# 66RING/tiny-flash-attention

Hardware: AMD Instinct MI355X
Metric: fwd TFLOPS + achieved %MFMA-roofline, (B=4,H=32,N=4096,D=128) bf16 (higher is better)
Workload: dtype bf16

## Files before the change

tiny-flash-attention_amd/csrc/tfa_fwd_il_epilogue.inc:

```
    if (PREF && !PREF2 && more_passes) issue_prologue(next_mb, true);
    if (SEAM) { seam_in = seam; if (seam) issue_prologue(next_mb, false); }
    typedef __attribute__((address_space(4))) const KArgs kargs_c;
    kargs_c* pe_ = (kargs_c*)__builtin_amdgcn_kernarg_segment_ptr();
    asm volatile("" : "+s"(pe_));
    kargs_c& pe = *pe_;
    VarSeq vse{};
    if constexpr (VARLEN) vse = varlen_seq(pe, b);
    const int lane_e = (int)__builtin_amdgcn_mbcnt_hi(~0u, __builtin_amdgcn_mbcnt_lo(~0u, 0u));
    const int qi_e = lane_e & 31, hi_e = lane_e >> 5, my_row_e = wave_row0 + qi_e;
    float l_tot = pair_sum((l4[0] + l4[1]) + (l4[2] + l4[3]));
    float w0 = 1.f, w1 = 0.f;
    const char* const dump = smem + 4 * TILE_BYTES;
    if constexpr (KSPLIT) {
      float* const ml = reinterpret_cast<float*>(smem + wave * (32 * D * 2)) + lane_e * 2;
      if (grp == 1) {
        ml[0] = mref; ml[1] = l_tot;
#pragma unroll
        for (int d = 0; d < DT; ++d) {
          float o[16];
          if (d == 0) o_read<0>(o, 1.f); else if (d == 1) o_read<1>(o, 1.f); else if (d == 2) o_read<2>(o, 1.f); else o_read<3>(o, 1.f);
#pragma unroll
          for (int g = 0; g < 4; ++g) {
            const f32x4 v4 = {o[4 * g + 0], o[4 * g + 1], o[4 * g + 2], o[4 * g + 3]};
            *reinterpret_cast<f32x4*>(const_cast<char*>(dump) + ((((wave * DT + d) << 2) + g) << 10) + lane_e * 16) = v4;
          }
        }
      }
      asm volatile("s_waitcnt lgkmcnt(0)\n\ts_barrier" ::: "memory");
      if (grp == 1) {
        if (!more_passes) return;
        asm volatile("s_barrier" ::: "memory");
        continue;
      }
      const float m1 = ml[0], l1 = ml[1];
      const float m = fmaxf(mref, m1);
      w0 = (mref == -INFINITY) ? 0.f : fast_exp2(mref - m);
      w1 = (m1 == -INFINITY) ? 0.f : fast_exp2(m1 - m);
      l_tot = w0 * l_tot + w1 * l1;
      mref = m;
    }
    const bool empty = !(l_tot > 0.f);
    const float inv = empty ? 1.f : 1.f / l_tot;
    auto o_get = [&](int d, float (&o)[16]) {
      const float f0 = inv * w0;
      if (d == 0) o_read<0>(o, f0); else if (d == 1) o_read<1>(o, f0); else if (d == 2) o_read<2>(o, f0); else o_read<3>(o, f0);
      if constexpr (KSPLIT) {
        const float f1 = inv * w1;
#pragma unroll
        for (int g = 0; g < 4; ++g) {
          const f32x4 x = *reinterpret_cast<const f32x4*>(dump + ((((wave * DT + d) << 2) + g) << 10) + lane_e * 16);
#pragma unroll
          for (int e = 0; e < 4; ++e) o[4 * g + e] = fmaf(f1, x[e], o[4 * g + e]);
        }
      }
    };
    if (PREF2) {
      const float lse = empty ? INFINITY : (mref + __builtin_amdgcn_logf(l_tot)) * 0.6931471805599453f;
      auto lse_rs = __builtin_amdgcn_make_buffer_rsrc((void*)(VARLEN ? pe.lse + ((long long)h * pe.total_q + vse.q0) : pe.lse + (long long)bh * pe.Nq), 0,
                                                      pe.lse != nullptr ? (unsigned)(VARLEN ? vse.nq : pe.Nq) * 4u : 0u, 0x00020000);
      __builtin_amdgcn_raw_buffer_store_b32(__builtin_bit_cast(unsigned, lse), lse_rs, hi_e == 0 ? my_row_e * 4 : (int)TFA_OOB, 0, 0);
    } else
    if (pe.lse != nullptr && hi_e == 0 && my_row_e < (VARLEN ? vse.nq : pe.Nq)) {
      const float lse = empty ? INFINITY : (mref + __builtin_amdgcn_logf(l_tot)) * 0.6931471805599453f;
      if constexpr (VARLEN) pe.lse[(long long)h * pe.total_q + vse.q0 + my_row_e] = lse;
      else pe.lse[(long long)bh * pe.Nq + my_row_e] = lse;
    }
    if (PREF2 && more_passes && !early_done) {
      asm volatile("" ::: "memory");
      issue_prologue(next_mb, true);
      asm volatile("" ::: "memory");
    }
    if (F32OUT) {
      float* obase = reinterpret_cast<float*>(pe.o) + (VARLEN ? (long long)vse.q0 * pe.os_n : b * pe.os_b) + h * pe.os_h;
      auto o_rs = slice_rsrc(obase, VARLEN ? varlen_bytes(vse.nq, pe.os_n, pe.dv, 4) : pe.o_bytes, (unsigned long long)q0 * (unsigned long long)pe.os_n * 4ull);
      const int ooff = (my_row_e - (WIN ? q0 : 0)) * (int)pe.os_n * 4 + hi_e * 16;
      static_assert(!F32OUT || NST_EPI == DT * 4, "NST_EPI must equal the fp32 epilogue's store count");
#pragma unroll
      for (int d = 0; d < DT; ++d) {
        float o[16];
        o_get(d, o);
#pragma unroll
        for (int g = 0; g < 4; ++g) {
// ... 67 lines not shown
```

tiny-flash-attention_amd/csrc/tfa_fwd_il_pass_prologue.inc:

```
    if (SEAM && seam_in) {  }
    else if (PREF2) {  }
    else if (QLDS && pass == 0) { issue_first(mb); asm volatile("s_setprio 0" ::: "memory"); }
    else if (!PREF || pass == 0) { issue_prologue(mb, true); asm volatile("s_setprio 0" ::: "memory"); }
    const bool seam = SEAM && (pass + 1 < npass) && ((nt & 1) == 0) && nt >= 2;
    if (!PREF2) o_zero<DT>();

    if (PREF2) {
    } else {
#if defined(TFA_IL_TRACEPRO)
      if (P_TRACE && pass == 0) {
        tp_issue = __builtin_amdgcn_s_memtime();
        asm volatile("s_waitcnt vmcnt(%0)" ::"n"(DS) : "memory");
        tp_kv = __builtin_amdgcn_s_memtime();
        asm volatile("s_waitcnt vmcnt(0)" ::: "memory");
        tp_q = __builtin_amdgcn_s_memtime();
      }
#endif
      if (QLDS && pass == 0) { wait_first(); read_q_lds(); }
      else asm volatile("s_waitcnt vmcnt(0)" ::: "memory");
#pragma unroll
      for (int s = 0; s < DS; ++s) asm volatile("" : "+v"(qf[s]));
    }
#if defined(TFA_IL_TRACEPRO)
    if (P_TRACE && pass == 0) tp_bar = __builtin_amdgcn_s_memtime();
#endif
    asm volatile("s_barrier" ::: "memory");
    if (P_TRACE && pass == tr_pass) t_pro = __builtin_amdgcn_s_memtime();

    const int nact = (wave_last_tile + 1 < nt_own) ? (wave_last_tile + 1) : nt_own;
    const bool idle_wave = (VF & VF_IL_IDLE) != 0 && wave_row0 >= p.Nq;
    int fm = nact;
    {
      int first_g = 0x3fffffff;
      if (IL_NK % BN) first_g = IL_NK / BN;
      if (CAUSAL) {
        const int c = pos_lo + shift + 1;
        const int full = c > 0 ? c / BN : 0;
        first_g = full < first_g ? full : first_g;
      }
      const int first = KSPLIT ? (first_g <= grp ? 0 : (first_g - grp + 1) >> 1) : first_g;
      fm = first < fm ? first : fm;
    }

    f32x16 sA[2], sB[2];
    asm volatile("" : "=v"(sA[0]), "=v"(sA[1]), "=v"(sB[0]), "=v"(sB[1]));
    float mA = -INFINITY, mB = -INFINITY;
    auto qk_burst = [&](int kbuf, int t, f32x16 (&s)[2], float& mout) {
#pragma unroll
      for (int tt = 0; tt < 2; ++tt)
#pragma unroll
        for (int r = 0; r < 16; ++r) s[tt][r] = 0.f;
      const unsigned kb = kbuf * TILE_BYTES;
#pragma unroll
      for (int i = 0; i < N1; ++i) s[KT(i)] = E::mfma(k_frag_rt(kb, i), qf[KS(i)], s[KT(i)]);
      if constexpr (SMOD) apply_bias(t, s);
      if (needs_mask(t)) apply_mask(t, s);
      float mx = s[0][0];
#pragma unroll
      for (int tt = 0; tt < 2; ++tt)
#pragma unroll
        for (int r = 0; r < 16; ++r) mx = fmaxf(mx, s[tt][r]);
      mout = pair_max(mx);
    };
    if (nact > 0 && !idle_wave) {
      qk_burst(0, 0, sA, mA);
      mref = fmaxf(mref, mA * sc);
    }
    if constexpr (MAXFREE) {
      if (seeded) {
        const int l_ = (int)__builtin_amdgcn_mbcnt_hi(~0u, __builtin_amdgcn_mbcnt_lo(~0u, 0u));
        mref = fmaxf(mref, reinterpret_cast<volatile float*>(smem + SEED_OFF)[wave_id * 32 + (l_ & 31)]);
      }
    }
    if (QLDS && pass == 0) asm volatile("s_waitcnt vmcnt(0)" ::: "memory");
    asm volatile("s_waitcnt lgkmcnt(0)\n\ts_barrier" ::: "memory");

#if defined(TFA_IL_TRACEWAIT)
    auto iter_end = [&]() {
      const unsigned long long a0 = __builtin_amdgcn_s_memtime();
      asm volatile("s_waitcnt vmcnt(0) lgkmcnt(0)" ::: "memory");
      const unsigned long long a1 = __builtin_amdgcn_s_memtime();
      asm volatile("s_barrier" ::: "memory");
      const unsigned long long a2 = __builtin_amdgcn_s_memtime();
      tw_wait += a1 - a0;
      tw_bar += a2 - a1;
    };
#elif defined(TFA_IL_TRACEITER)
    int it_n = 0;
    auto it_stamp = [&](int tag) {
      if (P_TRACE && pass == tr_pass && it_n < 16) {
        typedef __attribute__((address_space(3))) u32x2 lds_u32x2;
        const u32x2 rec = {(unsigned)__builtin_amdgcn_s_memtime(), (unsigned)tag};
        *reinterpret_cast<lds_u32x2*>(q_slice + it_n * 8) = rec;
        ++it_n;
      }
    };
    it_stamp(0);
    auto iter_end = [&]() { asm volatile("s_waitcnt vmcnt(0) lgkmcnt(0)\n\ts_barrier" ::: "memory"); it_stamp(2); };
#else
    auto iter_end = [&]() { asm volatile("s_waitcnt vmcnt(0) lgkmcnt(0)\n\ts_barrier" ::: "memory"); };
#endif
```

tiny-flash-attention_amd/csrc/tfa_fwd_il_tile_loop.inc:

```
    auto fused = [&](auto par_c, auto mask_c, auto resc_c, float alpha, int j, f32x16 (&scur)[2], f32x16 (&snext)[2], float& mnext) {
      constexpr int PAR = decltype(par_c)::value;
      constexpr bool MASK = decltype(mask_c)::value;
      constexpr bool RESC = decltype(resc_c)::value;
      static_assert(!RESC || N1 * 4 == 16 * DT, "one O register quad per QK^T MFMA");
      constexpr bool SPREAD = (VF & VF_IL_DMASPREAD) != 0;
      constexpr bool STAGGER = SPREAD && (VF & VF_IL_DMASTAGGER) != 0;
      const bool late = STAGGER && wave >= NW / 2;
      const bool issue_k = (j + 2 < nt) || seam;
      const int tk = (j + 2 < nt) ? j + 2 : j + 2 - nt;
      if (!SPREAD && !(AB & ILAB_NODMA)) {
        if (issue_k) dma_k(tk, PAR);
        dma_v(j + 1, PAR ^ 1);
      }
      const float msc = mref;
      constexpr int KB = PAR ^ 1;
      const char* vbp = vl + PAR * TILE_BYTES;
      unsigned pw[16];
      float xs[32];
      X8 kf[N1], vf[N2];
#pragma unroll
      for (int i = 0; i < PFK; ++i) kf[i] = k_frag(KB, i);
      auto soft_slot = [&](int g) {
#pragma unroll
        for (int e = 0; e < 32; ++e) {
// ... 132 lines not shown
        const int nact_s = __builtin_amdgcn_readfirstlane(nact), nt_s = __builtin_amdgcn_readfirstlane(nt);
        const int fmx = __builtin_amdgcn_readfirstlane(tail_on ? fm : -1);
        int ts;
        const int slim = __builtin_amdgcn_readfirstlane(wave_row0 + shift - key0_of(fm));
        constexpr bool BF = std::is_same<T, __bf16>::value;
        if constexpr (MAXFREE) {
          if constexpr (D == 128 && PPW == 2) { TFA_IL_ASM_LAZY_STMT(TFA_IL_ASM_LOOP_MF); }
          else if constexpr (D == 128) { TFA_IL_ASM_LAZY_STMT_G(TFA_IL_ASM_LOOP_D128_P4_MF, TFA_IL_ASM_Q8, TFA_IL_ASM_SRC4); }
          else if constexpr (PPW == 1) { TFA_IL_ASM_LAZY_STMT_G(TFA_IL_ASM_LOOP_D64_P1_MF, TFA_IL_ASM_Q4, TFA_IL_ASM_SRC1); }
          else { TFA_IL_ASM_LAZY_STMT_G(TFA_IL_ASM_LOOP_D64_P2_MF, TFA_IL_ASM_Q4, TFA_IL_ASM_SRC2); }
        }
        else if constexpr (D == 128 && PPW == 2 && BF) { TFA_IL_ASM_LAZY_STMT(TFA_IL_ASM_LOOP); }
        else if constexpr (D == 128 && PPW == 2) { TFA_IL_ASM_LAZY_STMT(TFA_IL_ASM_LOOP_F16); }
        else if constexpr (D == 128 && BF) { TFA_IL_ASM_LAZY_STMT_G(TFA_IL_ASM_LOOP_D128_P4, TFA_IL_ASM_Q8, TFA_IL_ASM_SRC4); }
        else if constexpr (D == 128) { TFA_IL_ASM_LAZY_STMT_G(TFA_IL_ASM_LOOP_D128_P4_F16, TFA_IL_ASM_Q8, TFA_IL_ASM_SRC4); }
        else if constexpr (PPW == 1 && BF) { TFA_IL_ASM_LAZY_STMT_G(TFA_IL_ASM_LOOP_D64_P1, TFA_IL_ASM_Q4, TFA_IL_ASM_SRC1); }
        else if constexpr (PPW == 1) { TFA_IL_ASM_LAZY_STMT_G(TFA_IL_ASM_LOOP_D64_P1_F16, TFA_IL_ASM_Q4, TFA_IL_ASM_SRC1); }
        else if constexpr (BF) { TFA_IL_ASM_LAZY_STMT_G(TFA_IL_ASM_LOOP_D64_P2, TFA_IL_ASM_Q4, TFA_IL_ASM_SRC2); }
        else { TFA_IL_ASM_LAZY_STMT_G(TFA_IL_ASM_LOOP_D64_P2_F16, TFA_IL_ASM_Q4, TFA_IL_ASM_SRC2); }
      }
    };
    auto asm_loop_exact = [&](int& j) {
      if constexpr (ASMLOOPX) {
        const int lim = fm < nact ? fm : nact;
        const int jend = (lim - 1 < nt_full - 2) ? lim - 1 : nt_full - 2;
        int koff = (j + 2) * k_tile_stride, voff = (j + 1) * v_tile_stride;
        const unsigned vaddr = lds_base + (unsigned)v_rd_base;
        const unsigned ldsw = __builtin_amdgcn_readfirstlane(lds_base + wave * (PPW * 1024));
        float alpha;
        u32x4 f0, f1, f2, f3, ka;
        unsigned ka5, ka6, ka7;
        const int nact_s = __builtin_amdgcn_readfirstlane(nact), nt_s = __builtin_amdgcn_readfirstlane(nt);
        const int fmx = __builtin_amdgcn_readfirstlane(tail_on ? fm : -1);
        int ts;
        const int slim = __builtin_amdgcn_readfirstlane(wave_row0 + shift - key0_of(fm));
        if constexpr (std::is_same<T, __bf16>::value) { TFA_IL_ASM_EXACT_STMT(TFA_IL_ASM_LOOP_EXACT); }
        else { TFA_IL_ASM_EXACT_STMT(TFA_IL_ASM_LOOP_EXACT_F16); }
      }
    };
    if (!idle_wave)
#pragma nounroll
    for (int j = 0; j < nact; j += 2) {
      if constexpr (EXACT) {
        if (ASMLOOPX && (loop_ok(j) || tail_on)) {
          int jj = j;
          asm_loop_exact(jj);
          if (jj & 1) j = jj - 1;
          else { j = jj - 2; continue; }
        } else
        if (j + 1 < nact) fast_exact(C0{}, j + 1 >= fm, j, sA, mA, sB, mB);
        else slow(j, sA, mA, sB, mB);
        if (j + 1 >= nact) break;
        if (j + 2 < nact) fast_exact(C1{}, j + 2 >= fm, j + 1, sB, mB, sA, mA);
        else slow(j + 1, sB, mB, sA, mA);
      } else {
      if (ASMLOOP && !trigger(mA) && (loop_ok(j) || tail_on) && (!LOCAL || j + 1 >= nlm)) {
        int jj = j;
        asm_loop(jj, (early_ok && nact == nt) ? 1 : 0);
#if defined(TFA_IL_TRACEITER)
        it_stamp(1 | (jj << 8));
#endif
        if (jj & 1) j = jj - 1;
        else { j = jj - 2; continue; }
      } else
      if (!ASMLOOP && j + 1 < nact && !trigger(mA)) {
        if (SMOD ? !needs_mask(j + 1) : j + 1 < fm) fused(C0{}, MN{}, MN{}, 1.f, j, sA, sB, mB);
        else fused(C0{}, MY{}, MN{}, 1.f, j, sA, sB, mB);
      } else {
        slow(j, sA, mA, sB, mB);
      }
      if (j + 1 >= nact) break;
      if (ASMLOOP && early_ok && nact == nt && j + 1 == nt - 1 && !trigger(mB)) {
        last_pending = true;
        break;
      }
      if (!ASMLOOP && j + 2 < nact && !trigger(mB)) {
        if (SMOD ? !needs_mask(j + 2) : j + 2 < fm) fused(C1{}, MN{}, MN{}, 1.f, j + 1, sB, sA, mA);
        else fused(C1{}, MY{}, MN{}, 1.f, j + 1, sB, sA, mA);
      } else {
        slow(j + 1, sB, mB, sA, mA);
      }
      }
    }
#pragma nounroll
    for (int j = idle_wave ? 0 : (last_pending ? nt - 1 : nact); j < nt; ++j) {
      if (early_ok && j == nt - 1) {
        issue_early(block_of(pass + 1));
        early_done = true;
        if (last_pending) {
          int jj = j;
          asm_loop(jj, 2);
        } else asm volatile("s_waitcnt lgkmcnt(0)\n\ts_barrier" ::: "memory");
#if defined(TFA_IL_TRACEITER)
        it_stamp(2);
#endif
        break;
      }
      if (j + 2 < nt) dma_k(j + 2, j & 1);
      else if (seam) dma_k(j + 2 - nt, j & 1);
      if (j + 1 < nt) dma_v(j + 1, (j & 1) ^ 1);
      else if (seam) dma_v(0, (j & 1) ^ 1);
      iter_end();
    }
    bool redo_pass = false;
    if constexpr (MAXFREE) {
      volatile int* const redo_w = reinterpret_cast<volatile int*>(smem + REDO_OFF);
      const float lt_ = (l4[0] + l4[1]) + (l4[2] + l4[3]);
      if (__any(!(lt_ <= 0x1p64f))) *redo_w = 1;
      asm volatile("s_waitcnt lgkmcnt(0)\n\ts_barrier" ::: "memory");
      redo_pass = __builtin_amdgcn_readfirstlane(*redo_w) != 0 && !seeded;
      seeded = false;
    }
    if (P_TRACE && pass == tr_pass) t_loop = __builtin_amdgcn_s_memtime();
#if defined(TFA_IL_TRACEITER)
    if (P_TRACE && pass == tr_pass && blockIdx.x < 64) {
      typedef __attribute__((address_space(3))) const u32x2 lds_u32x2c;
      it_stamp(3 | (nt << 8) | (nact << 16));
      const int l_ = (int)__builtin_amdgcn_mbcnt_hi(~0u, __builtin_amdgcn_mbcnt_lo(~0u, 0u));
      if (l_ < 16) {
        const u32x2 r_ = *reinterpret_cast<lds_u32x2c*>(q_slice + l_ * 8);
        P_TRACE[(size_t)gridDim.x * 8 + ((size_t)blockIdx.x * 8 + wave_id) * 16 + l_] = l_ < it_n ? (((unsigned long long)r_[1] << 32) | r_[0]) : 0ull;
      }
      asm volatile("s_waitcnt vmcnt(0) lgkmcnt(0)" ::: "memory");
    }
#endif
```

tiny-flash-attention_amd/csrc/tfa_fwd_kernel_il.h:

```cpp
#pragma once
#include <type_traits>
#include "tfa_fwd_kernel_dma.h"

namespace tfa {


constexpr int VF_IL = 32768;
constexpr int VF_IL_DMASPREAD = 65536;
constexpr int VF_IL_EPI = 262144;
constexpr int VF_IL_EPI_INPLACE = 1048576;
constexpr int VF_IL_PREF = 524288;
constexpr int VF_IL_SEAM = 2097152;
constexpr int VF_IL_KSPLIT = 1 << 25;
constexpr int VF_IL_IDLE = 1 << 26;
constexpr bool IL_DECODE_NT = true;
constexpr int IL_OSTORE_AUX = 2;
constexpr int VF_IL_WINDOWED = 1 << 24;
constexpr int VF_IL_PREF2 = 1 << 29;
constexpr int VF_IL_QLDS = 1 << 28;
constexpr int VF_IL_EXACT = 1 << 30;
constexpr int VF_IL_DMASTAGGER = 131072;
constexpr int VF_IL_VARLEN = 1 << 23;
constexpr int VF_IL_LOCAL = 1 << 22;
constexpr int VF_IL_ALIBI = 256;
constexpr int VF_IL_SOFTCAP = 512;

}
#include "tfa_fwd_il_regs.h"
#if defined(TFA_IL_ASM_INC)
#include TFA_IL_ASM_INC
#else
#include "tfa_fwd_il_asm_loop.inc"
#endif
#define TFA_IL_ASM_Q8 [q0] "v"(qf[0]), [q1] "v"(qf[1]), [q2] "v"(qf[2]), [q3] "v"(qf[3]), [q4] "v"(qf[4]), [q5] "v"(qf[5]), [q6] "v"(qf[6]), [q7] "v"(qf[7])
#define TFA_IL_ASM_Q4 [q0] "v"(qf[0]), [q1] "v"(qf[1]), [q2] "v"(qf[2]), [q3] "v"(qf[3])
#define TFA_IL_ASM_SRC1 [ks0] "v"(k_src[0]), [vs0] "v"(v_src[0])
#define TFA_IL_ASM_SRC2 [ks0] "v"(k_src[0]), [ks1] "v"(k_src[1]), [vs0] "v"(v_src[0]), [vs1] "v"(v_src[1])
#define TFA_IL_ASM_SRC4 [ks0] "v"(k_src[0]), [ks1] "v"(k_src[1]), [ks2] "v"(k_src[2]), [ks3] "v"(k_src[3]), [vs0] "v"(v_src[0]), [vs1] "v"(v_src[1]), [vs2] "v"(v_src[2]), [vs3] "v"(v_src[3])
#define TFA_IL_ASM_LAZY_STMT_G(TEXT, QOPS, SRCOPS) \
  asm volatile(TEXT \
  : [sa0] "+v"(sA[0]), [sa1] "+v"(sA[1]), [sb0] "+v"(sB[0]), [sb1] "+v"(sB[1]), \
  [l0] "+v"(l4[0]), [l1] "+v"(l4[1]), [l2] "+v"(l4[2]), [l3] "+v"(l4[3]), [ma] "+v"(mA), [mb] "+v"(mB), [j] "+s"(j), \
  [koff] "+s"(koff), [voff] "+s"(voff), [ts] "=&s"(ts), \
  [f0] "=&v"(f0), [f1] "=&v"(f1), [f2] "=&v"(f2), [f3] "=&v"(f3), [ka] "=&v"(ka), [ka5] "=&v"(ka5), [ka6] "=&v"(ka6), [ka7] "=&v"(ka7), [thr] "=&v"(thr) \
  : QOPS, [mref] "v"(mref), [kaddr] "v"(k_rd_addr), [va] "v"(vaddr), SRCOPS, \
  [sc] "s"(sc), [krs] "s"(k_rs), [vrs] "s"(v_rs), [ldsw] "s"(ldsw), [kstr] "s"(k_tile_stride), [vstr] "s"(v_tile_stride), [jend] "s"(jend), \
  [nact] "s"(nact_s), [fmx] "s"(fmx), [nt] "s"(nt_s), [slim] "s"(slim), [xl] "s"(xl) \
  : TFA_O_CLOB0, TFA_O_CLOB1, TFA_O_CLOB2, TFA_O_CLOB3, "m0", "vcc", "scc", "memory")
#define TFA_IL_ASM_LAZY_STMT(TEXT) TFA_IL_ASM_LAZY_STMT_G(TEXT, TFA_IL_ASM_Q8, TFA_IL_ASM_SRC2)
#define TFA_IL_ASM_EXACT_STMT(TEXT) \
  asm volatile(TEXT \
  : [sa0] "+v"(sA[0]), [sa1] "+v"(sA[1]), [sb0] "+v"(sB[0]), [sb1] "+v"(sB[1]), \
  [l0] "+v"(l4[0]), [l1] "+v"(l4[1]), [l2] "+v"(l4[2]), [l3] "+v"(l4[3]), [ma] "+v"(mA), [mb] "+v"(mB), [mref] "+v"(mref), [j] "+s"(j), \
  [koff] "+s"(koff), [voff] "+s"(voff), [ts] "=&s"(ts), \
  [f0] "=&v"(f0), [f1] "=&v"(f1), [f2] "=&v"(f2), [f3] "=&v"(f3), [ka] "=&v"(ka), [ka5] "=&v"(ka5), [ka6] "=&v"(ka6), [ka7] "=&v"(ka7), [alpha] "=&v"(alpha) \
  : [q0] "v"(qf[0]), [q1] "v"(qf[1]), [q2] "v"(qf[2]), [q3] "v"(qf[3]), [q4] "v"(qf[4]), [q5] "v"(qf[5]), [q6] "v"(qf[6]), [q7] "v"(qf[7]), \
  [kaddr] "v"(k_rd_addr), [va] "v"(vaddr), [ks0] "v"(k_src[0]), [ks1] "v"(k_src[1]), [vs0] "v"(v_src[0]), [vs1] "v"(v_src[1]), \
  [sc] "s"(sc), [krs] "s"(k_rs), [vrs] "s"(v_rs), [ldsw] "s"(ldsw), [kstr] "s"(k_tile_stride), [vstr] "s"(v_tile_stride), [jend] "s"(jend), \
  [nact] "s"(nact_s), [fmx] "s"(fmx), [nt] "s"(nt_s), [slim] "s"(slim) \
  : TFA_O_CLOB0, TFA_O_CLOB1, TFA_O_CLOB2, TFA_O_CLOB3, "m0", "vcc", "scc", "memory")
#if !defined(TFA_IL_USE_ASMTAIL)
#define TFA_IL_USE_ASMTAIL 1
#endif
#if !defined(TFA_IL_USE_EARLY)
#define TFA_IL_USE_EARLY 0
#endif
#if !defined(TFA_IL_USE_MAXFREE)
#define TFA_IL_USE_MAXFREE 1
#endif
#if !defined(TFA_IL_USE_ASMLOOP)
#define TFA_IL_USE_ASMLOOP 1
#endif

#if defined(TFA_IL_PAD)
#define TFA_IL_PAD1_0 asm volatile("s_nop 0");
#define TFA_IL_PAD1_1 { int pad_s_; asm volatile("s_mov_b32 %0, 0" : "=s"(pad_s_)); }
#define TFA_IL_PAD1_2 { int pad_v_; asm volatile("v_mov_b32 %0, 0" : "=v"(pad_v_)); }
#define TFA_IL_PAD1_3 asm volatile("s_waitcnt vmcnt(63) lgkmcnt(15)");
#define TFA_IL_PADCAT_(k) TFA_IL_PAD1_##k
#define TFA_IL_PADCAT(k) TFA_IL_PADCAT_(k)
#define TFA_IL_PAD_HERE { _Pragma("unroll") for (int pad_i_ = 0; pad_i_ < TFA_IL_PAD; ++pad_i_) TFA_IL_PADCAT(TFA_IL_PADKIND) }
#else
#define TFA_IL_PAD_HERE
#endif

namespace tfa {

constexpr int ILAB_TRACE = 256;
#define P_TRACE ((AB & ILAB_TRACE) ? p.trace : (unsigned long long*)nullptr)
constexpr int ILAB_NOEXP = 1, ILAB_NODMA = 2, ILAB_NOBARRIER = 4, ILAB_NOMAX = 8, ILAB_NOQK = 16, ILAB_NOPV = 32, ILAB_NOKREAD = 64, ILAB_NOVREAD = 128;

template <typename T, int D, int NW, bool CAUSAL, bool F32OUT, int VF, int AB = 0, int DVB = D / 32>
__global__ __launch_bounds__(NW * 64, 2) __attribute__((amdgpu_num_vgpr(96))) void fwd_kernel_il(const KArgs p) {
  using E = Elem<T>;
  using X8 = typename E::x8;
  constexpr bool KSPLIT = (VF & VF_IL_KSPLIT) != 0;
  constexpr int NWG = KSPLIT ? NW / 2 : NW;
  constexpr int BM = NWG * 32;
  static_assert(!KSPLIT || ((VF & VF_IL_EPI_INPLACE) && !(VF & (VF_IL_SEAM | VF_IL_PREF | VF_IL_WINDOWED))), "KSPLIT: in-place epilogue");
  constexpr int KSTEP = KSPLIT ? 2 : 1;
  constexpr int BN = 64;
  constexpr int CPR = D / 8;
  constexpr int TILE_BYTES = BN * D * 2;
  constexpr int PIECES = TILE_BYTES / 1024;
  constexpr int PPW = PIECES / NWG;
  static_assert(DVB >= 1 && DVB <= D / 32, "valid 32-column blocks of a D-wide kernel");
  constexpr int DS = 2 * DVB;
  constexpr int DT = DVB;
  constexpr int DT_L = D / 32;
  constexpr int N1 = 2 * DS;
  constexpr int N2 = 4 * DT;
  constexpr int NE1 = 21;
  constexpr int PFK = 2, PFV = 2;
  auto slot_of_elem = [](int e) constexpr -> int {
    return 1 + (e < NE1 ? e * N1 / NE1 : N1 + (e - NE1) * (3 * DT - 1) / (32 - NE1));
  };
  static_assert(slot_of_elem(7) < N1 && slot_of_elem(15) < N1 + DT && slot_of_elem(23) < N1 + 2 * DT && slot_of_elem(31) < N1 + 3 * DT,
                "a P slot is packed too late for the PV MFMA that reads it");
#define KT(i) ((i) & 1)
#define KS(i) ((i) >> 1)
  constexpr bool PAIR = CAUSAL && (VF & VF_PAIR);
  static_assert(PPW >= 1 && PPW * NWG == PIECES, "tile does not split into whole DMA pieces per wave");

  extern __shared__ __attribute__((aligned(1024))) char smem[];
  asm volatile("s_setprio 1" ::: "memory");
  const int wave_id = __builtin_amdgcn_readfirstlane(threadIdx.x >> 6);
  const int grp = KSPLIT ? wave_id / NWG : 0;
  char* const gsm = smem + grp * 4 * TILE_BYTES;
  char* const kl = gsm;
  char* const vl = gsm + 2 * TILE_BYTES;
  const unsigned lds_base = (unsigned)(size_t)(__attribute__((address_space(3))) char*)gsm;

  unsigned long long t_start = 0, t_pro = 0, t_loop = 0, rt_start = 0;
#if defined(TFA_IL_TRACEPRO)
  const unsigned long long tp_entry = __builtin_amdgcn_s_memtime();
#endif
  if (P_TRACE) { rt_start = __builtin_amdgcn_s_memrealtime(); t_start = __builtin_amdgcn_s_memtime(); }
  const int tid = threadIdx.x;
  const int lane = tid & 63;
#if defined(TFA_IL_TRACEPRO)
#define TP_STAMP(k, dep)                                                                                                         \
  do {                                                                                                                             \
    asm volatile("" ::"s"(dep));                                                                                                   \
    if (P_TRACE) {                                                                                                                 \
      const unsigned long long t_ = __builtin_amdgcn_s_memtime();                                                                  \
      P_TRACE[(size_t)gridDim.x * 8 + (size_t)gridDim.x * 32 + ((size_t)blockIdx.x * 8 + wave_id) * 8 + (k)] = t_;  \
    }                                                                                                                              \
  } while (0)
  if (P_TRACE) P_TRACE[(size_t)gridDim.x * 8 + (size_t)gridDim.x * 32 + ((size_t)blockIdx.x * 8 + wave_id) * 8 + 0] = tp_entry;
// ... 94 lines not shown
    v_bytes = v_bytes > vo ? v_bytes - vo : 0;
  }
  auto slice_rsrc = [&](const void* base, unsigned long long bytes, unsigned long long off) {
    if constexpr (WIN) return rsrc_at(base, bytes, off);
    else return __builtin_amdgcn_make_buffer_rsrc((void*)base, 0, (unsigned)bytes, 0x00020000);
  };
  auto k_rs = __builtin_amdgcn_make_buffer_rsrc((void*)kbase, 0, WIN ? 0u : (unsigned)k_bytes, 0x00020000);
  auto v_rs = __builtin_amdgcn_make_buffer_rsrc((void*)vbase, 0, WIN ? 0u : (unsigned)v_bytes, 0x00020000);

  int k_src[PPW], v_src[PPW];
#pragma unroll
  for (int i = 0; i < PPW; ++i) {
    const int pc = wave * PPW + i;
    {
      const int row = pc * (1024 / (D * 2)) + lane / CPR;
      const int cpos = lane % CPR;
      const int kch = cpos ^ k_swz<D>(row);
      k_src[i] = kch * 8 < p.dv ? row * (int)p.ks_n * 2 + (kch << 4) : (int)TFA_OOB;
    }
    {
      const int o = pc * 1024 + lane * 16;
      const int sub = o >> 9, R = (o >> 6) & 7, pcs = (o >> 4) & 3;
      const int dt = sub % DT_L, sh = sub / DT_L;
      const int key = 16 * (sh >> 1) + 4 * (sh & 1) + 8 * (R >> 2) + (R & 3);
      v_src[i] = (dt * 4 + pcs) * 8 < p.dv ? key * (int)p.vs_n * 2 + ((dt * 4 + pcs) << 4) : (int)TFA_OOB;
    }
  }
  const int k_tile_stride = (KSPLIT ? 2 : 1) * BN * (int)p.ks_n * 2;
  const int v_tile_stride = (KSPLIT ? 2 : 1) * BN * (int)p.vs_n * 2;

  TP_STAMP(2, (int)(size_t)qbase + (int)(size_t)kbase + (int)(size_t)vbase);
  const bool kv_private = p.H == p.Hk && p.kv_stream != 0;
  auto dma_k1 = [&](int t, int buf, int i) {
    if constexpr (WIN) lds_dma16_m0_fresh(rsrc_at(kbase, k_bytes, (unsigned long long)t * (unsigned)k_tile_stride), lds_base + buf * TILE_BYTES + (wave * PPW + i) * 1024, k_src[i]);
    else if ((VF & VF_IL_IDLE) && IL_DECODE_NT && kv_private) lds_dma16_m0_nt(k_rs, lds_base + buf * TILE_BYTES + (wave * PPW + i) * 1024, k_src[i] + t * k_tile_stride);
    else lds_dma16_m0(k_rs, lds_base + buf * TILE_BYTES + (wave * PPW + i) * 1024, k_src[i] + t * k_tile_stride);
  };
  auto dma_v1 = [&](int t, int buf, int i) {
    if constexpr (WIN) lds_dma16_m0_fresh(rsrc_at(vbase, v_bytes, (unsigned long long)t * (unsigned)v_tile_stride), lds_base + (2 + buf) * TILE_BYTES + (wave * PPW + i) * 1024, v_src[i]);
    else if ((VF & VF_IL_IDLE) && IL_DECODE_NT && kv_private) lds_dma16_m0_nt(v_rs, lds_base + (2 + buf) * TILE_BYTES + (wave * PPW + i) * 1024, v_src[i] + t * v_tile_stride);
    else lds_dma16_m0(v_rs, lds_base + (2 + buf) * TILE_BYTES + (wave * PPW + i) * 1024, v_src[i] + t * v_tile_stride);
  };
  auto dma_k = [&](int t, int buf) {
#pragma unroll
    for (int i = 0; i < PPW; ++i) dma_k1(t, buf, i);
  };
  auto dma_v = [&](int t, int buf) {
#pragma unroll
    for (int i = 0; i < PPW; ++i) dma_v1(t, buf, i);
  };

  unsigned k_rd_addr = lds_base + qi * (D * 2) + ((hi ^ k_swz<D>(qi)) << 4);
  asm volatile("" : "+v"(k_rd_addr));
  const int i16 = lane & 15, g16 = (lane >> 4) & 1;
  const int v_rd_base = (hi * DT_L << 9) + ((i16 >> 2) << 6) + (g16 << 5) + ((i16 & 3) << 3);
  const float sc = p.scale_log2;
  int nt_total = 0, n_slow = 0;
  unsigned long long tw_wait = 0, tw_bar = 0;

#if defined(TFA_IL_TRACEPRO)
  asm volatile("" ::"v"(k_src[0]), "v"(v_src[PPW - 1]));
#endif
  TP_STAMP(3, wi);
  const int npass = PAIR ? ((nmb_x - 1 - wi) != wi ? 2 : 1) : 1;
  constexpr bool EPI = (VF & VF_IL_EPI) != 0;
  constexpr bool PREF2 = PAIR && (VF & VF_IL_PREF2) != 0;
  constexpr bool QLDS = (VF & VF_IL_QLDS) != 0;
  constexpr bool EXACT = (VF & VF_IL_EXACT) != 0;
  constexpr bool MAXFREE_BASE = std::is_same<T, __bf16>::value && !EXACT && !LOCAL && TFA_IL_USE_MAXFREE && TFA_IL_USE_ASMLOOP && (D == 128 || D == 64) && DVB == D / 32 &&
                                (AB & ~ILAB_TRACE) == 0 && !(VF & (VF_IL_WINDOWED | VF_IL_IDLE | VF_IL_DMASTAGGER | VF_IL_SEAM)) && (PPW == 1 || PPW == 2 || PPW == 4);
  constexpr bool MAXFREE = MAXFREE_BASE;
  static_assert(!MAXFREE || !((VF & VF_IL_PREF) && !(VF & VF_IL_PREF2)), "max-free: a redone pass re-issues its own first requests (PREF2 or no prefetch)");
  constexpr int REDO_OFF = (KSPLIT ? 8 : 4) * TILE_BYTES + (((VF & VF_IL_EPI) && !(VF & VF_IL_EPI_INPLACE)) ? NW * 32 * D * 2 : 0);
  constexpr int SEED_OFF = REDO_OFF + 16;
  bool seeded = false;
  if (MAXFREE && threadIdx.x == 0) *reinterpret_cast<volatile int*>(smem + REDO_OFF) = 0;
  static_assert(!QLDS || ((VF & VF_IL_EPI) && !(VF & (VF_IL_EPI_INPLACE | VF_IL_KSPLIT | VF_IL_WINDOWED | VF_IL_IDLE | VF_IL_SEAM))), "QLDS: a wave-private slice of the separate epilogue region");
  constexpr int NST_EPI = F32OUT ? 4 * DT : ((VF & VF_IL_EPI) ? 32 / (64 / (D / 8)) : 4 * DT);
  constexpr bool PREF = (VF & VF_IL_PREF) != 0 || PREF2;
  static_assert(!PREF2 || ((VF & VF_IL_EPI) && !(VF & (VF_IL_EPI_INPLACE | VF_IL_SEAM | VF_IL_KSPLIT))), "PREF2: separate epilogue region, no seam streaming");
  constexpr bool SEAM = PAIR && (VF & VF_IL_SEAM) != 0;
  static_assert(!(SEAM && PREF), "SEAM includes the Q prefetch");
  static_assert(!(SEAM && (VF & VF_IL_EPI_INPLACE)), "the in-place epilogue would overwrite the streamed tiles");
  bool seam_in = false;
  X8 qf[DS];
  auto own_tiles = [&](int ntg) -> int { return KSPLIT ? (ntg - grp + 1) >> 1 : ntg; };
  auto key0_of = [&](int t) -> int { return (KSTEP * t + grp) * BN; };
  auto block_of = [&](int pass) -> int {
    if (PAIR) return pass == 0 ? (nmb_x - 1 - wi) : wi;
    return CAUSAL ? (nmb_x - 1 - wi) : wi;
  };
  typedef __attribute__((address_space(4))) const KArgs kargs_c;
  auto fresh_args = [&]() -> kargs_c* {
    kargs_c* a_ = (kargs_c*)__builtin_amdgcn_kernarg_segment_ptr();
    asm volatile("" : "+s"(a_));
    return a_;
  };
  auto issue_prologue = [&](int mbx, bool with_dma) {
    kargs_c& p = *fresh_args();
    VarSeq vx{};
    if constexpr (VARLEN) vx = varlen_seq(p, b);
    const int q0x = mbx * BM;
    int kve = (VARLEN ? vx.nk : p.Nk) - (LOCAL ? kofs : 0);
    if (CAUSAL) {
      const int lim = (((VF & VF_IL_IDLE) && p.row_mod > 0) ? p.row_mod : q0x + BM) + shift;
      kve = lim < kve ? lim : kve;
    }
    const int ntx = own_tiles(kve > 0 ? (kve + BN - 1) / BN : 0);
    if (with_dma && ntx > 0) dma_k(0, 0);
    if (with_dma && ntx > 0) dma_v(0, 0);
    int one = 1;
    asm volatile("" : "+s"(one));
    if (with_dma && ntx > 1) dma_k(one, 1);
    auto q_rs = slice_rsrc(qbase, VARLEN ? varlen_bytes(vx.nq, p.qs_n, p.dv, 2) : p.q_bytes, (unsigned long long)q0x * (unsigned long long)p.qs_n * 2ull);
    const int lane_p = (int)__builtin_amdgcn_mbcnt_hi(~0u, __builtin_amdgcn_mbcnt_lo(~0u, 0u));
    int hix = lane_p >> 5;
    asm volatile("" : "+v"(hix));
    const int qoff = ((WIN ? 0 : q0x) + wrow * 32 + (lane_p & 31)) * (int)p.qs_n * 2 + hix * 16;
#pragma unroll
    for (int s = 0; s < DS; ++s) {
      u32x4 t = __builtin_amdgcn_raw_buffer_load_b128(q_rs, (2 * s + hix) * 8 < p.dv ? qoff + s * 32 : (int)TFA_OOB, 0, 0);
      qf[s] = __builtin_bit_cast(X8, t);
    }
  };
  auto issue_early = [&](int mbx) {
    kargs_c& p = *fresh_args();
    dma_k(0, 0);
    dma_v(0, 0);
    int one = 1;
    asm volatile("" : "+s"(one));
    dma_k(one, 1);
    const int q0x = mbx * BM;
    auto q_rs = slice_rsrc(qbase, p.q_bytes, (unsigned long long)q0x * (unsigned long long)p.qs_n * 2ull);
    const int lane_p = (int)__builtin_amdgcn_mbcnt_hi(~0u, __builtin_amdgcn_mbcnt_lo(~0u, 0u));
    int hix = lane_p >> 5;
    asm volatile("" : "+v"(hix));
    const int qoff = ((WIN ? 0 : q0x) + wrow * 32 + (lane_p & 31)) * (int)p.qs_n * 2 + hix * 16;
    asm volatile("s_nop 4" ::: "memory");
#pragma unroll
    for (int s = 0; s < DS; ++s) {
      const int off = (2 * s + hix) * 8 < p.dv ? qoff + s * 32 : (int)TFA_OOB;
      asm volatile("buffer_load_dwordx4 %0, %1, %2, 0 offen" : "+v"(qf[s]) : "v"(off), "s"(q_rs) : "memory");
    }
  };
  const unsigned q_slice = lds_base + 4 * TILE_BYTES + wave * (32 * D * 2);
  auto issue_q_dma = [&](int mbx) {
    constexpr int RPP = 1024 / (D * 2);
    auto q_rs = slice_rsrc(qbase, VARLEN ? varlen_bytes(vsq.nq, p.qs_n, p.dv, 2) : p.q_bytes, 0ull);
    const int r0 = __builtin_amdgcn_readfirstlane(mbx * BM + wave * 32);
#pragma unroll
    for (int i = 0; i < 32 / RPP; ++i) {
      const int row = i * RPP + lane / CPR, cpos = lane % CPR;
      const int kch = cpos ^ k_swz<D>(row);
      const int off = kch * 8 < p.dv ? (r0 + row) * (int)p.qs_n * 2 + (kch << 4) : (int)TFA_OOB;
      lds_dma16_m0(q_rs, __builtin_amdgcn_readfirstlane(q_slice) + i * 1024, off);
    }
  };
  auto read_q_lds = [&]() {
    typedef __attribute__((address_space(3))) const u32x4 lds_u32x4;
#pragma unroll
    for (int s = 0; s < DS; ++s) {
      const unsigned a = q_slice + qi * (D * 2) + ((((2 * s + hi) ^ k_swz<D>(qi))) << 4);
      qf[s] = __builtin_bit_cast(X8, *reinterpret_cast<lds_u32x4*>(a));
    }
  };
  int first_late = 0;
// ... 279 lines not shown
```

tiny-flash-attention_amd/csrc/tfa_launch.h:

```cpp
#pragma once
#include <hip/hip_runtime.h>
#include "tfa_host_util.h"
#include "tfa_fwd_kernel.h"
#include "tfa_fwd_kernel_dma.h"
#include "tfa_fwd_kernel_il.h"
#include "tfa_fwd_kernel_x4.h"
#if defined(TFA_EXPERIMENTAL)
#include "tfa_fwd_kernel_bringup.h"
#include "tfa_fwd_kernel_pp.h"
#include "tfa_fwd_kernel_swp.h"
#include "tfa_fwd_kernel_w64.h"
#endif

namespace tfa {

struct Variant {
  int id;
  const char* name;
  int nw;
  int vf;
  int rb;
};

constexpr int kDefaultVariant = 30;
constexpr int kSmallGridVariant = 32;
constexpr int kX4D256Variant = 34;
constexpr int kKSplitVariant = 36;
constexpr int kKSplitPairVariant = 37;
constexpr int kExactVariant = 38;
constexpr int kSplitVariant = 17;
static const Variant kVariants[] = {
    {17, "dma4-pair-2buf (LDS-DMA, burst-structured, exact running max; 128-row blocks, two LDS buffers: two workgroups per CU)", 4, VF_DMA | VF_PAIR | VF_2BUF, 1},
    {30, "il8-pair-dmaspread-epi (issue-interleaved, 8 waves; O leaves through a separate LDS region as whole rows, 16-byte stores; causal pairs: the light "
         "pass is requested before the heavy pass's O stores; a workgroup's first Q rows arrive through LDS)", 8,
     VF_DMA | VF_IL | VF_PAIR | VF_IL_DMASPREAD | VF_IL_EPI | VF_IL_PREF2 | VF_IL_QLDS, 1},
    {32, "il4-pair-epi (4 waves x2 workgroups per CU; O leaves through the idle tile buffers as whole rows)", 4, VF_DMA | VF_IL | VF_PAIR | VF_IL_EPI | VF_IL_EPI_INPLACE, 1},
    {34, "x4-d256-pair (the x4 kernel with ONE 32-row block per wave: head dims 136..256, 128-row workgroups, O leaves through the idle tile buffers as whole rows)", 4, VF_DMA | VF_IL | VF_X4 | VF_PAIR, 1},
    {36, "il8-ksplit-epi (small grids: 8 waves on one 128-row block, waves 0-3 take the even KV tiles and waves 4-7 the odd ones, merged through LDS)", 8,
     VF_DMA | VF_IL | VF_IL_DMASPREAD | VF_IL_EPI | VF_IL_EPI_INPLACE | VF_IL_KSPLIT, 1},
    {37, "il8-ksplit-pair-epi (the key-split kernel with causal blocks paired heavy+light per workgroup: two 128-row blocks per CU)", 8,
     VF_DMA | VF_IL | VF_PAIR | VF_IL_DMASPREAD | VF_IL_EPI | VF_IL_EPI_INPLACE | VF_IL_KSPLIT, 1},
    {38, "exact-il8-pair-dmaspread-epi (variant 30's kernel with the EXACT running row maximum — the reference's rounding points of P, TFA_FWD_EXACT_MAX on grids "
         "that fill the chip: tiles in which some row of a wave saw a new maximum run a body that also re-bases O behind the QK^T MFMAs)", 8,
     VF_DMA | VF_IL | VF_PAIR | VF_IL_DMASPREAD | VF_IL_EPI | VF_IL_PREF2 | VF_IL_QLDS | VF_IL_EXACT, 1},
};
constexpr int kNumProductVariants = sizeof(kVariants) / sizeof(kVariants[0]);

constexpr int kX4Variant = 33;
constexpr int kSeamVariant = 35;
#if defined(TFA_EXPERIMENTAL)
static const Variant kExperimentalVariants[] = {
    {0, "w8-gatherV (bring-up: 16-bit LDS gathers for V, no transpose read)", 8, 0, 1},
    {1, "w8-trV (8 waves x 32 rows, ds_read_b64_tr_b16 for V)", 8, VF_TRREAD, 1},
    {2, "w4-trV (4 waves x 32 rows, 2 workgroups/CU)", 4, VF_TRREAD, 1},
    {3, "w8-trV-alwaysrescale (no exact alpha==1 skip)", 8, VF_TRREAD | VF_NOSKIP, 1},
    {4, "w8-trV-pair (causal blocks paired heavy+light per workgroup)", 8, VF_TRREAD | VF_PAIR, 1},
    {5, "w8-trV-pair-kpre-vpre (K and V fragments prefetched to registers)", 8, VF_TRREAD | VF_PAIR | VF_KPRE | VF_VPRE, 1},
    {6, "w4-trV-pair-kpre-vpre", 4, VF_TRREAD | VF_PAIR | VF_KPRE | VF_VPRE, 1},
    {7, "w8-trV-pair-vpre", 8, VF_TRREAD | VF_PAIR | VF_VPRE, 1},
    {8, "pp8-pair-vpre0 (ping-pong: two wave groups half a tile apart; V fragments read in the 2nd half)", 8, VF_PP | VF_PAIR | (0 << VF_VPRE_SHIFT), 1},
    {9, "pp8-pair-vpre2 (ping-pong; V fragments of 2 d-tiles read ahead in the 1st half)", 8, VF_PP | VF_PAIR | (2 << VF_VPRE_SHIFT), 1},
    {10, "pp8-pair-vpre4 (ping-pong; all V fragments read ahead in the 1st half)", 8, VF_PP | VF_PAIR | (4 << VF_VPRE_SHIFT), 1},
    {11, "dma8-pair (LDS-DMA staging, 3 tile buffers, counted vmcnt; 8 waves)", 8, VF_DMA | VF_PAIR, 1},
    {12, "dma4-pair (LDS-DMA staging, 3 tile buffers; 4 waves, 1 workgroup/CU by LDS)", 4, VF_DMA | VF_PAIR, 1},
    {13, "dma8-pair-setprio", 8, VF_DMA | VF_PAIR | VF_PRIO, 1},
    {14, "swp8-pair (LDS-DMA + software-pipelined loop: softmax(j) beside QK^T(j+1), PV(j) beside rowmax(j+1))", 8, VF_DMA | VF_SWP | VF_PAIR, 1},
    {15, "dma8-pair-persistent (256 workgroups walk the work items; next block prefetched behind the epilogue)", 8, VF_DMA | VF_PAIR | VF_PERSIST, 1},
    {16, "dma4-pair-persistent (128-row blocks, 256 persistent workgroups)", 4, VF_DMA | VF_PAIR | VF_PERSIST, 1},
    {18, "dma4-pair-2buf-persistent", 4, VF_DMA | VF_PAIR | VF_2BUF | VF_PERSIST, 1},
    {19, "dma8-pair-2buf (two LDS buffers, prefetch distance one tile)", 8, VF_DMA | VF_PAIR | VF_2BUF, 1},
    {20, "w64-pair (4 waves x 64 rows, one wave per SIMD, O accumulators pinned in AGPRs by inline-asm MFMA)", 4, VF_DMA | VF_W64 | VF_PAIR, 2},
    {21, "dma4-pair-2buf-ldsepi (O leaves through LDS as whole rows, 16-byte stores)", 4, VF_DMA | VF_PAIR | VF_2BUF | VF_LDSEPI, 1},
    {22, "dma8-pair-2buf-ldsepi", 8, VF_DMA | VF_PAIR | VF_2BUF | VF_LDSEPI, 1},
    {23, "pp8-vpre4-gapqk8 (ping-pong + 8-cycle issue gap behind every QK^T MFMA)", 8, VF_PP | VF_PAIR | (4 << VF_VPRE_SHIFT) | (8 << VF_NOPQK_SHIFT), 1},
    {24, "pp8-vpre4-gapqk8-gappv8", 8, VF_PP | VF_PAIR | (4 << VF_VPRE_SHIFT) | (8 << VF_NOPQK_SHIFT) | (8 << VF_NOPPV_SHIFT), 1},
    {25, "pp8-vpre4-gapqk16", 8, VF_PP | VF_PAIR | (4 << VF_VPRE_SHIFT) | (16 << VF_NOPQK_SHIFT), 1},
    {26, "il8-pair (issue-interleaved: every MFMA followed by its share of another tile's softmax; 8 waves)", 8, VF_DMA | VF_IL | VF_PAIR, 1},
    {27, "il4-pair (issue-interleaved, 4 waves, two workgroups per CU)", 4, VF_DMA | VF_IL | VF_PAIR, 1},
    {28, "il8-pair-dmaspread (LDS-DMA pieces issued between the first QK^T MFMAs)", 8, VF_DMA | VF_IL | VF_PAIR | VF_IL_DMASPREAD, 1},
    {29, "il8-pair-dmastagger (waves 4-7 issue their LDS-DMA pieces behind the first PV MFMAs instead)", 8, VF_DMA | VF_IL | VF_PAIR | VF_IL_DMASPREAD | VF_IL_DMASTAGGER, 1},
    {31, "il8-pair-dmaspread-epi-pref (+ the next pass's first tiles and Q requested before the epilogue, vmcnt(0) in the prologue)", 8, VF_DMA | VF_IL | VF_PAIR | VF_IL_DMASPREAD | VF_IL_EPI | VF_IL_PREF, 1},
    {33, "il-x4-pair-epi (issue-interleaved, 4 waves x 64 rows: one wave per SIMD, O and Q in AGPRs, K ring of three LDS buffers)", 4, VF_DMA | VF_IL | VF_X4 | VF_PAIR | VF_X4_EPI, 2},
    {35, "il8-pair-dmaspread-epi-seam (the heavy pass's last tiles stream the light pass's K(0), K(1), V(0); Q before the epilogue)", 8, VF_DMA | VF_IL | VF_PAIR | VF_IL_DMASPREAD | VF_IL_EPI | VF_IL_SEAM, 1},
};
constexpr int kNumExperimentalVariants = sizeof(kExperimentalVariants) / sizeof(kExperimentalVariants[0]);
#endif
constexpr int kNumVariants = 39;

static inline const Variant* variant_info(int variant) {
  for (int i = 0; i < kNumProductVariants; ++i)
    if (kVariants[i].id == variant) return &kVariants[i];
#if defined(TFA_EXPERIMENTAL)
  for (int i = 0; i < kNumExperimentalVariants; ++i)
    if (kExperimentalVariants[i].id == variant) return &kExperimentalVariants[i];
#endif
  return nullptr;
}
static inline bool variant_built(int variant) { return variant_info(variant) != nullptr; }

struct LaunchGeom {
  int grid, block, lds;
};

template <int D, int NW, int VF>
constexpr int il_lds_bytes() {
  return ((VF & VF_IL_KSPLIT) ? 8 : 4) * 64 * D * 2 + (((VF & VF_IL_EPI) && !(VF & VF_IL_EPI_INPLACE)) ? NW * 32 * D * 2 : 0) + 16 + NW * 32 * 4;
}

template <typename T, int D, bool CAUSAL>
hipError_t launch_fwd_c(const KArgs& a, bool f32out, int variant, hipStream_t stream, LaunchGeom* geom, bool dry);
#define TFA_FWD_UNITS(T, D)                                                                             \
  template <> hipError_t launch_fwd_c<T, D, false>(const KArgs&, bool, int, hipStream_t, LaunchGeom*, bool); \
  template <> hipError_t launch_fwd_c<T, D, true>(const KArgs&, bool, int, hipStream_t, LaunchGeom*, bool);
TFA_FWD_UNITS(__bf16, 64) TFA_FWD_UNITS(__bf16, 128) TFA_FWD_UNITS(_Float16, 64) TFA_FWD_UNITS(_Float16, 128)
#undef TFA_FWD_UNITS
template <typename T, int D>
static inline hipError_t launch_fwd(const KArgs& a, bool causal, bool f32out, int variant, hipStream_t stream, LaunchGeom* geom, bool dry) {
// ... 123 lines not shown
```

Before: 1132.

## Store finished waves' O rows early on the causal diagonal tiles

In the default causal paired kernel, a wave whose rows have seen all their keys on the diagonal now runs its epilogue at that point: it normalizes O, writes the LSE, and stores O through its private LDS slice. The remaining waves keep processing the last tiles while those stores are in flight. At pass end the early wave skips the normal epilogue and only issues the next pass's prologue and zeroes O. The cost is extra code and register pressure in the tile loop, plus an added vmcnt/barrier wait inside the loop.

```diff
diff --git a/tiny-flash-attention_amd/csrc/tfa_fwd_il_epilogue.inc b/tiny-flash-attention_amd/csrc/tfa_fwd_il_epilogue.inc
--- a/tiny-flash-attention_amd/csrc/tfa_fwd_il_epilogue.inc
+++ b/tiny-flash-attention_amd/csrc/tfa_fwd_il_epilogue.inc
@@ -1,3 +1,15 @@
+    if constexpr (EARLY_EPI) {
+      if (stored_early) {
+        if (more_passes) {
+          issue_prologue(next_mb, true);
+          o_zero<DT>();
+        }
+        asm volatile("s_waitcnt vmcnt(0)" ::: "memory");
+#pragma unroll
+        for (int s = 0; s < DS; ++s) asm volatile("" : "+v"(qf[s]));
+        continue;
+      }
+    }
     if (PREF && !PREF2 && more_passes) issue_prologue(next_mb, true);
     if (SEAM) { seam_in = seam; if (seam) issue_prologue(next_mb, false); }
     typedef __attribute__((address_space(4))) const KArgs kargs_c;
diff --git a/tiny-flash-attention_amd/csrc/tfa_fwd_il_pass_prologue.inc b/tiny-flash-attention_amd/csrc/tfa_fwd_il_pass_prologue.inc
--- a/tiny-flash-attention_amd/csrc/tfa_fwd_il_pass_prologue.inc
+++ b/tiny-flash-attention_amd/csrc/tfa_fwd_il_pass_prologue.inc
@@ -87,11 +87,12 @@
     };
 #elif defined(TFA_IL_TRACEITER)
     int it_n = 0;
+    const unsigned it_base = EARLY_EPI ? lds_base + SEED_OFF + wave_id * 128 : q_slice;
     auto it_stamp = [&](int tag) {
       if (P_TRACE && pass == tr_pass && it_n < 16) {
         typedef __attribute__((address_space(3))) u32x2 lds_u32x2;
         const u32x2 rec = {(unsigned)__builtin_amdgcn_s_memtime(), (unsigned)tag};
-        *reinterpret_cast<lds_u32x2*>(q_slice + it_n * 8) = rec;
+        *reinterpret_cast<lds_u32x2*>(it_base + it_n * 8) = rec;
         ++it_n;
       }
     };
diff --git a/tiny-flash-attention_amd/csrc/tfa_fwd_il_tile_loop.inc b/tiny-flash-attention_amd/csrc/tfa_fwd_il_tile_loop.inc
--- a/tiny-flash-attention_amd/csrc/tfa_fwd_il_tile_loop.inc
+++ b/tiny-flash-attention_amd/csrc/tfa_fwd_il_tile_loop.inc
@@ -238,6 +238,67 @@
       }
       }
     }
+    bool stored_early = false;
+    auto early_epilogue = [&]() {
+      if constexpr (EARLY_EPI) {
+        kargs_c& pe = *fresh_args();
+        const int lane_e = (int)__builtin_amdgcn_mbcnt_hi(~0u, __builtin_amdgcn_mbcnt_lo(~0u, 0u));
+        const int qi_e = lane_e & 31, hi_e = lane_e >> 5, my_row_e = wave_row0 + qi_e;
+        const float l_tot = pair_sum((l4[0] + l4[1]) + (l4[2] + l4[3]));
+        const bool empty = !(l_tot > 0.f);
+        const float inv = empty ? 1.f : 1.f / l_tot;
+        auto o_get = [&](int d, float (&o)[16]) {
+          if (d == 0) o_read<0>(o, inv); else if (d == 1) o_read<1>(o, inv); else if (d == 2) o_read<2>(o, inv); else o_read<3>(o, inv);
+        };
+        const float lse = empty ? INFINITY : (mref + __builtin_amdgcn_logf(l_tot)) * 0.6931471805599453f;
+        auto lse_rs = __builtin_amdgcn_make_buffer_rsrc((void*)(pe.lse + (long long)bh * pe.Nq), 0, pe.lse != nullptr ? (unsigned)pe.Nq * 4u : 0u, 0x00020000);
+        __builtin_amdgcn_raw_buffer_store_b32(__builtin_bit_cast(unsigned, lse), lse_rs, hi_e == 0 ? my_row_e * 4 : (int)TFA_OOB, 0, 0);
+        if constexpr (F32OUT) {
+          float* obase = reinterpret_cast<float*>(pe.o) + b * pe.os_b + h * pe.os_h;
+          auto o_rs = slice_rsrc(obase, pe.o_bytes, 0ull);
+          const int ooff = my_row_e * (int)pe.os_n * 4 + hi_e * 16;
+#pragma unroll
+          for (int d = 0; d < DT; ++d) {
+            float o[16];
+            o_get(d, o);
+#pragma unroll
+            for (int g = 0; g < 4; ++g) {
+              f32x4 v4 = {o[4 * g + 0], o[4 * g + 1], o[4 * g + 2], o[4 * g + 3]};
+              __builtin_amdgcn_raw_buffer_store_b128(__builtin_bit_cast(u32x4, v4), o_rs, d * 32 + g * 8 + hi_e * 4 < pe.dv ? ooff + (d * 32 + g * 8) * 4 : (int)TFA_OOB, 0, 0);
+            }
+          }
+        } else {
+          T* obase = reinterpret_cast<T*>(pe.o) + b * pe.os_b + h * pe.os_h;
+          auto o_rs = slice_rsrc(obase, pe.o_bytes, 0ull);
+          typedef __attribute__((ext_vector_type(4))) T t4;
+          int qix = qi_e, lanex = lane_e;
+          asm volatile("" : "+v"(qix), "+v"(lanex));
+          char* const ow = smem + 4 * TILE_BYTES + wave * (32 * D * 2);
+          constexpr int CH = D / 8;
+          const int osw = (CH == 16) ? (qix & 15) : (qix & 7);
+#pragma unroll
+          for (int d = 0; d < DT; ++d) {
+            float o[16];
+            o_get(d, o);
+#pragma unroll
+            for (int g = 0; g < 4; ++g) {
+              t4 v4 = {(T)o[4 * g + 0], (T)o[4 * g + 1], (T)o[4 * g + 2], (T)o[4 * g + 3]};
+              const int c = d * 4 + g;
+              *reinterpret_cast<u32x2*>(ow + qix * (D * 2) + ((c ^ osw) << 4) + (lanex >> 5) * 8) = __builtin_bit_cast(u32x2, v4);
+            }
+          }
+          asm volatile("s_waitcnt lgkmcnt(0)" ::: "memory");
+          constexpr int RPI = 64 / CH;
+#pragma unroll
+          for (int i = 0; i < 32 / RPI; ++i) {
+            const int r = i * RPI + lanex / CH, cpos = lanex % CH;
+            const int c = cpos ^ ((CH == 16) ? (r & 15) : (r & 7));
+            u32x4 v = *reinterpret_cast<const u32x4*>(ow + r * (D * 2) + (cpos << 4));
+            __builtin_amdgcn_raw_buffer_store_b128(v, o_rs, c * 8 < pe.dv ? (wave_row0 + r) * (int)pe.os_n * 2 + (c << 4) : (int)TFA_OOB, 0, IL_OSTORE_AUX);
+          }
+        }
+      }
+    };
 #pragma nounroll
     for (int j = idle_wave ? 0 : (last_pending ? nt - 1 : nact); j < nt; ++j) {
       if (early_ok && j == nt - 1) {
@@ -256,6 +317,17 @@
       else if (seam) dma_k(j + 2 - nt, j & 1);
       if (j + 1 < nt) dma_v(j + 1, (j & 1) ^ 1);
       else if (seam) dma_v(0, (j & 1) ^ 1);
+      if constexpr (EARLY_EPI) {
+        if (j == nact && !(fresh_args()->dbg & IL_DBG_NO_EARLY_EPI)) {
+          early_epilogue();
+          stored_early = true;
+          asm volatile("s_waitcnt vmcnt(%0) lgkmcnt(0)\n\ts_barrier" ::"n"(NST_EPI + 1) : "memory");
+#if defined(TFA_IL_TRACEITER)
+          it_stamp(2);
+#endif
+          continue;
+        }
+      }
       iter_end();
     }
     bool redo_pass = false;
@@ -274,7 +346,7 @@
       it_stamp(3 | (nt << 8) | (nact << 16));
       const int l_ = (int)__builtin_amdgcn_mbcnt_hi(~0u, __builtin_amdgcn_mbcnt_lo(~0u, 0u));
       if (l_ < 16) {
-        const u32x2 r_ = *reinterpret_cast<lds_u32x2c*>(q_slice + l_ * 8);
+        const u32x2 r_ = *reinterpret_cast<lds_u32x2c*>(it_base + l_ * 8);
         P_TRACE[(size_t)gridDim.x * 8 + ((size_t)blockIdx.x * 8 + wave_id) * 16 + l_] = l_ < it_n ? (((unsigned long long)r_[1] << 32) | r_[0]) : 0ull;
       }
       asm volatile("s_waitcnt vmcnt(0) lgkmcnt(0)" ::: "memory");
diff --git a/tiny-flash-attention_amd/csrc/tfa_fwd_kernel_il.h b/tiny-flash-attention_amd/csrc/tfa_fwd_kernel_il.h
--- a/tiny-flash-attention_amd/csrc/tfa_fwd_kernel_il.h
+++ b/tiny-flash-attention_amd/csrc/tfa_fwd_kernel_il.h
@@ -65,6 +65,9 @@
 #if !defined(TFA_IL_USE_EARLY)
 #define TFA_IL_USE_EARLY 0
 #endif
+#if !defined(TFA_IL_USE_EARLY_EPI)
+#define TFA_IL_USE_EARLY_EPI 1
+#endif
 #if !defined(TFA_IL_USE_MAXFREE)
 #define TFA_IL_USE_MAXFREE 1
 #endif
@@ -325,6 +328,10 @@
   constexpr bool SEAM = PAIR && (VF & VF_IL_SEAM) != 0;
   static_assert(!(SEAM && PREF), "SEAM includes the Q prefetch");
   static_assert(!(SEAM && (VF & VF_IL_EPI_INPLACE)), "the in-place epilogue would overwrite the streamed tiles");
+  constexpr bool EARLY_EPI = TFA_IL_USE_EARLY_EPI && !TFA_IL_USE_EARLY && PREF2 && NW == 8 && !VARLEN && (AB & ~ILAB_TRACE) == 0;
+  static_assert(!EARLY_EPI || (CAUSAL && EPI && !(VF & (VF_IL_EPI_INPLACE | VF_IL_KSPLIT | VF_IL_WINDOWED | VF_IL_IDLE | VF_IL_SEAM)) && !LOCAL),
+                "early epilogue: fixed-length paired causal blocks with a wave-private slice of the separate epilogue region");
+  constexpr int IL_DBG_NO_EARLY_EPI = 1024;
   bool seam_in = false;
   X8 qf[DS];
   auto own_tiles = [&](int ntg) -> int { return KSPLIT ? (ntg - grp + 1) >> 1 : ntg; };
diff --git a/tiny-flash-attention_amd/csrc/tfa_launch.h b/tiny-flash-attention_amd/csrc/tfa_launch.h
--- a/tiny-flash-attention_amd/csrc/tfa_launch.h
+++ b/tiny-flash-attention_amd/csrc/tfa_launch.h
@@ -32,7 +32,8 @@
 static const Variant kVariants[] = {
     {17, "dma4-pair-2buf (LDS-DMA, burst-structured, exact running max; 128-row blocks, two LDS buffers: two workgroups per CU)", 4, VF_DMA | VF_PAIR | VF_2BUF, 1},
     {30, "il8-pair-dmaspread-epi (issue-interleaved, 8 waves; O leaves through a separate LDS region as whole rows, 16-byte stores; causal pairs: the light "
-         "pass is requested before the heavy pass's O stores; a workgroup's first Q rows arrive through LDS)", 8,
+         "pass is requested before the heavy pass's O stores; a workgroup's first Q rows arrive through LDS; on the causal diagonal the waves that have finished "
+         "store their O rows under the tiles the others still run)", 8,
      VF_DMA | VF_IL | VF_PAIR | VF_IL_DMASPREAD | VF_IL_EPI | VF_IL_PREF2 | VF_IL_QLDS, 1},
     {32, "il4-pair-epi (4 waves x2 workgroups per CU; O leaves through the idle tile buffers as whole rows)", 4, VF_DMA | VF_IL | VF_PAIR | VF_IL_EPI | VF_IL_EPI_INPLACE, 1},
     {34, "x4-d256-pair (the x4 kernel with ONE 32-row block per wave: head dims 136..256, 128-row workgroups, O leaves through the idle tile buffers as whole rows)", 4, VF_DMA | VF_IL | VF_X4 | VF_PAIR, 1},
```

Result: slower. 1112 (-1.8%).
